# AutoGPTQ/AutoGPTQ

Measured on AMD Instinct MI355X. Metric: int4 g128 QuantLinear fwd GB/s + tokens/s, Llama-7B shapes, higher is better.
Workload: dtype f16; 1 GPU; Llama-7B linear shapes (4096->4096 x4, 4096->11008 x2, 11008->4096) x 32 blocks = 224 layers, int4 g128 no act-order, M=1 rows per step, 128 launches/step in one hipGraph (q|k|v and gate|up of a block: one gptq_forward_multi launch each); layers=224, launches=128, parallelism=single

## Files before the change

### autogptq_amd/_lib.py

```python
from __future__ import annotations

import ctypes
import os
from ctypes import POINTER, Structure, c_char_p, c_int, c_int32, c_size_t, c_void_p

import torch

_HERE = os.path.dirname(os.path.abspath(__file__))
LIB_PATH = os.environ.get("GPTQ_MI355X_LIB", os.path.join(_HERE, "libgptq_mi355x.so"))

ABI_VERSION = 8

GPTQ_F16, GPTQ_BF16, GPTQ_F32 = 0, 1, 2
ZERO_WRAP, ZERO_NOWRAP = 0, 1
EPI_NONE, EPI_SILU_MUL, EPI_GELU_TANH_MUL = 0, 1, 2
EPILOGUE_ENUM = {"none": EPI_NONE, "silu_mul": EPI_SILU_MUL, "gelu_tanh_mul": EPI_GELU_TANH_MUL}

DTYPE_ENUM = {torch.float16: GPTQ_F16, torch.bfloat16: GPTQ_BF16, torch.float32: GPTQ_F32}

EXPORTS = (
    "gptq_abi_version", "gptq_last_error", "gptq_status_string", "gptq_workspace_bytes", "gptq_workspace_bytes_ex",
    "gptq_forward", "gptq_forward_ex", "gptq_gemv", "gptq_gemm", "gptq_dequant", "gptq_grad_input",
    "gptq_unpack_weights", "gptq_unpack_zeros", "gptq_pack_weights", "gptq_pack_zeros",
    "gptq_make_sequential", "gptq_resequence_qweight", "gptq_permute_columns", "gptq_prepack_decode", "gptq_prepack_decode_bytes", "gptq_unprepack_decode",
    "gptq_awq_unpack", "gptq_awq_repack", "gptq_describe_plan",
    "gptq_init", "gptq_workspace_bytes_max", "gptq_validate_g_idx",
    "gptq_forward_multi", "gptq_workspace_bytes_multi", "gptq_forward_multi_ex", "gptq_workspace_bytes_multi_ex",
    "gptq_peer_scatter", "gptq_peer_collect", "gptq_peer_gather", "gptq_forward_scatter", "gptq_forward_gather", "gptq_peer_publish",
    "gptq_mlp_forward", "gptq_mlp_forward_ex", "gptq_mlp_forward_act", "gptq_workspace_bytes_mlp", "gptq_workspace_bytes_mlp_ex", "gptq_describe_mlp_plan",
    "gptq_moe_table_bytes", "gptq_moe_build_table", "gptq_moe_workspace_bytes", "gptq_moe_forward", "gptq_describe_moe_plan",
    "gptq_moe_decode_table_bytes", "gptq_moe_build_decode_table", "gptq_moe_decode_workspace_bytes", "gptq_moe_decode_forward", "gptq_describe_moe_decode_plan",
    "gptq_moe_batch_workspace_bytes", "gptq_moe_batch_forward", "gptq_describe_moe_batch_plan",
    "gptq_moe_prefill_workspace_bytes", "gptq_moe_prefill_forward", "gptq_describe_moe_prefill_plan",
    "gptq_moe_grad_table_bytes", "gptq_moe_build_grad_table", "gptq_moe_backward_workspace_bytes", "gptq_moe_backward", "gptq_describe_moe_backward_plan",
    "gptq_lora_down", "gptq_lora_up", "gptq_lora_apply", "gptq_describe_lora_plan",
    "gptq_lora_backward_workspace_bytes", "gptq_lora_backward", "gptq_describe_lora_backward_plan",
    "gptq_adapter_route_bytes", "gptq_adapter_route", "gptq_adapter_rows_apply", "gptq_describe_adapter_rows_plan",
    "gptq_moe_router", "gptq_describe_moe_router_plan", "gptq_moe_router_grouped", "gptq_describe_moe_router_grouped_plan",
    "gptq_moe_shared_decode_workspace_bytes", "gptq_moe_shared_decode_forward", "gptq_describe_moe_shared_decode_plan", "gptq_moe_shared_combine",
)
WS_HEADER_BYTES = 65536
STRIP_COLS = 16


class GptqLayer(Structure):
    _fields_ = [
        ("qweight", c_void_p), ("qzeros", c_void_p), ("scales", c_void_p), ("g_idx", c_void_p), ("bias", c_void_p),
        ("K", c_int32), ("N", c_int32), ("bits", c_int32), ("group_size", c_int32),
# ... 104 lines not shown
    lib.gptq_forward_multi.argtypes = [POINTER(POINTER(GptqLayer)), c_int, c_void_p, POINTER(c_void_p), c_int, c_void_p, c_size_t, c_void_p]
    lib.gptq_workspace_bytes_multi_ex.restype = c_size_t
    lib.gptq_workspace_bytes_multi_ex.argtypes = [POINTER(POINTER(GptqLayer)), c_int, c_int, POINTER(GptqTuning)]
    lib.gptq_forward_multi_ex.argtypes = lib.gptq_forward_multi.argtypes + [POINTER(GptqTuning)]
    lib.gptq_validate_g_idx.argtypes = [c_void_p, c_int, c_int]
    fw = [POINTER(GptqLayer), c_void_p, c_void_p, c_int, c_void_p, c_size_t, c_void_p]
    lib.gptq_forward.argtypes = fw
    for name in ("gptq_forward_ex", "gptq_gemv", "gptq_gemm"):
        getattr(lib, name).argtypes = fw + [POINTER(GptqTuning)]
    lib.gptq_dequant.argtypes = [POINTER(GptqLayer), c_void_p, c_void_p]
    lib.gptq_grad_input.argtypes = [POINTER(GptqLayer), c_void_p, c_void_p, c_int, c_int, c_void_p]
    lib.gptq_unpack_weights.argtypes = [c_void_p, c_int, c_int, c_int, c_void_p, c_void_p]
    lib.gptq_unpack_zeros.argtypes = [c_void_p, c_int, c_int, c_int, c_int, c_void_p, c_void_p]
    lib.gptq_pack_weights.argtypes = [c_void_p, c_void_p, c_void_p, c_void_p, c_int, c_int, c_int, c_int, c_int, c_int,
                                      c_void_p, c_void_p, c_void_p]
    lib.gptq_pack_zeros.argtypes = [c_void_p, c_int, c_int, c_int, c_int, c_void_p, c_void_p]
    lib.gptq_make_sequential.argtypes = [c_void_p, c_int, c_int, c_void_p, POINTER(c_int)]
    lib.gptq_resequence_qweight.argtypes = [c_void_p, c_void_p, c_int, c_int, c_int, c_void_p, c_void_p]
    lib.gptq_permute_columns.argtypes = [c_void_p, c_void_p, c_int, c_int, c_int, c_void_p, c_void_p]
    lib.gptq_prepack_decode_bytes.argtypes = [POINTER(GptqLayer), POINTER(c_size_t), POINTER(c_size_t)]
    lib.gptq_prepack_decode.argtypes = [POINTER(GptqLayer), c_void_p, c_void_p, c_void_p]
    lib.gptq_unprepack_decode.argtypes = [c_void_p, c_int, c_int, c_int, c_void_p, c_void_p]
    lib.gptq_describe_plan.argtypes = [POINTER(GptqLayer), c_int, POINTER(GptqTuning), c_char_p, c_size_t]
    lib.gptq_awq_unpack.argtypes = [c_void_p, c_void_p, c_void_p, c_int, c_int, c_int, c_void_p, c_void_p, c_void_p]
    lib.gptq_awq_repack.argtypes = [c_void_p, c_void_p, c_int, c_int, c_int, c_void_p, c_void_p, c_void_p]
    LP = POINTER(GptqLayer)
    lib.gptq_workspace_bytes_mlp.restype = c_size_t
    lib.gptq_workspace_bytes_mlp.argtypes = [LP, LP, LP, c_int]
    lib.gptq_workspace_bytes_mlp_ex.restype = c_size_t
    lib.gptq_workspace_bytes_mlp_ex.argtypes = [LP, LP, LP, c_int, POINTER(GptqTuning)]
    lib.gptq_mlp_forward.argtypes = [LP, LP, LP, c_void_p, c_void_p, c_int, c_void_p, c_size_t, c_void_p]
    lib.gptq_mlp_forward_ex.argtypes = lib.gptq_mlp_forward.argtypes + [POINTER(GptqTuning)]
    lib.gptq_mlp_forward_act.argtypes = [LP, LP, LP, c_int, c_void_p, c_void_p, c_int, c_void_p, c_size_t, c_void_p]
    lib.gptq_describe_mlp_plan.argtypes = [LP, LP, LP, c_int, POINTER(GptqTuning), c_char_p, c_size_t]
    MP = POINTER(GptqMoe)
    lib.gptq_moe_table_bytes.restype = c_size_t
    lib.gptq_moe_table_bytes.argtypes = [c_int]
    lib.gptq_moe_build_table.argtypes = [MP, c_void_p, c_void_p]
    lib.gptq_moe_workspace_bytes.restype = c_size_t
    lib.gptq_moe_workspace_bytes.argtypes = [MP, c_int, c_int]
    lib.gptq_moe_forward.argtypes = [MP, c_void_p, c_void_p, c_void_p, c_void_p, c_int, c_int, c_void_p, c_void_p, c_void_p, c_size_t, c_void_p]
    lib.gptq_describe_moe_plan.argtypes = [MP, c_int, c_int, c_char_p, c_size_t]
    lib.gptq_moe_decode_table_bytes.restype = c_size_t
    lib.gptq_moe_decode_table_bytes.argtypes = [c_int]
    lib.gptq_moe_build_decode_table.argtypes = [MP, c_void_p, c_void_p]
    lib.gptq_moe_decode_workspace_bytes.restype = c_size_t
# ... 106 lines not shown
def check(status: int) -> None:
    if status != 0:
        lib = load()
        msg = lib.gptq_last_error().decode("utf-8", "replace")
        kind = lib.gptq_status_string(status).decode()
        raise GptqError(status, f"gptq_mi355x: {kind}: {msg}")


def _describe(fn: str, *args) -> dict:
    buf = ctypes.create_string_buffer(512)
    check(getattr(load(), fn)(*args, buf, len(buf)))
    out = {}
    for kv in buf.value.decode().split():
        k, v = kv.split("=", 1)
        out[k] = int(v) if v.lstrip("-").isdigit() else v
    return out


def _pointer_array(ctype, items):
    return (POINTER(ctype) * max(1, len(items)))(*[ctypes.pointer(i) for i in items])


def describe_plan(layer: "GptqLayer", M: int, tuning: "GptqTuning | None" = None) -> dict:
    return _describe("gptq_describe_plan", ctypes.byref(layer), M, ctypes.byref(tuning) if tuning is not None else None)


def describe_mlp_plan(gate: "GptqLayer", up: "GptqLayer", down: "GptqLayer", M: int, tuning: "GptqTuning | None" = None) -> dict:
    return _describe("gptq_describe_mlp_plan", ctypes.byref(gate), ctypes.byref(up), ctypes.byref(down), M,
                     ctypes.byref(tuning) if tuning is not None else None)


def describe_moe_plan(moe: "GptqMoe", T: int, topk: int) -> dict:
    return _describe("gptq_describe_moe_plan", ctypes.byref(moe), T, topk)


def describe_moe_backward_plan(moe: "GptqMoe", T: int, topk: int) -> dict:
    return _describe("gptq_describe_moe_backward_plan", ctypes.byref(moe), T, topk)


def describe_moe_decode_plan(moe: "GptqMoe", T: int, topk: int) -> dict:
    return _describe("gptq_describe_moe_decode_plan", ctypes.byref(moe), T, topk)


def describe_moe_shared_decode_plan(moe: "GptqMoe", shared: "GptqMoeShared", T: int, topk: int) -> dict:
    return _describe("gptq_describe_moe_shared_decode_plan", ctypes.byref(moe), ctypes.byref(shared), T, topk)


# ... 53 lines not shown
```

### autogptq_amd/csrc/capi.hip

```cpp
#include <stdarg.h>
#include <stdio.h>
#include <string.h>

#include <algorithm>
#include <cstdlib>
#include <vector>

#include "common.cuh"
#include "launch.h"
#include "../../include/gptq_mi355x_lab.h"

using namespace gptq;

namespace {

thread_local char g_err[512] = "";

int fail(int code, const char* fmt, ...) {
    va_list ap;
    va_start(ap, fmt);
    vsnprintf(g_err, sizeof(g_err), fmt, ap);
    va_end(ap);
    return code;
}
// ... 1500 lines not shown
    if (e != hipSuccess) return hip_fail(e, "gptq_prepack_decode launch");
    return GPTQ_OK;
}

int gptq_unprepack_decode(const uint32_t* qweight_tiled, int K, int N, int bits, uint32_t* qweight_out, void* stream) {
    if (!qweight_tiled || !qweight_out) return fail(GPTQ_ERR_NULL, "qweight_tiled/qweight_out must be non-NULL");
    if (bits != 2 && bits != 3 && bits != 4 && bits != 8) return fail(GPTQ_ERR_UNSUPPORTED, "the decode copy exists for 2-, 3-, 4- and 8-bit layers (got %d)", bits);
    if (K <= 0 || N <= 0 || K % 32 || N % GPTQ_STRIP_COLS) return fail(GPTQ_ERR_SHAPE, "K (%d) must be a positive multiple of 32 and N (%d) of %d", K, N, GPTQ_STRIP_COLS);
    if ((const void*)qweight_tiled == (const void*)qweight_out) return fail(GPTQ_ERR_UNSUPPORTED, "gptq_unprepack_decode does not work in place");
    hipError_t e = launch_unprepack_decode(qweight_tiled, K, N, bits, qweight_out, (hipStream_t)stream);
    if (e != hipSuccess) return hip_fail(e, "gptq_unprepack_decode launch");
    return GPTQ_OK;
}

int gptq_permute_columns(const void* x, const int32_t* perm, int M, int K, int dtype, void* x_out, void* stream) {
    if (!x || !perm || !x_out) return fail(GPTQ_ERR_NULL, "x/perm/x_out must be non-NULL");
    if (!dtype_ok(dtype)) return fail(GPTQ_ERR_UNSUPPORTED, "unsupported dtype enum %d", dtype);
    if (M <= 0 || K <= 0) return fail(GPTQ_ERR_SHAPE, "M (%d) and K (%d) must be > 0", M, K);
    hipError_t e = launch_permute_columns(x, perm, M, K, dtype, x_out, (hipStream_t)stream);
    if (e != hipSuccess) return hip_fail(e, "gptq_permute_columns launch");
    return GPTQ_OK;
}

int gptq_describe_plan(const gptq_layer_t* L, int M, const gptq_tuning_t* tune, char* out, size_t out_bytes) {
    if (!out || out_bytes == 0) return fail(GPTQ_ERR_NULL, "out must be non-NULL");
    out[0] = 0;
    int rc = check_layer(L);
    if (rc) return rc;
    if (M <= 0) return fail(GPTQ_ERR_SHAPE, "M must be > 0, got %d", M);
    if (tune && (tune->path == 2 || tune->path == 4)) return fail(GPTQ_ERR_UNSUPPORTED, "tuning.path = %d was retired in round 6", tune->path);
    const ForwardRoute r = route_forward(L, M, tune);
    const char* separate = r.unfused_epilogue ? "separate" : "none";
    switch (r.kind) {
        case ROUTE_TILED:
        case ROUTE_TILED_PAIR: {
            const bool pair = r.kind == ROUTE_TILED_PAIR;
            snprintf(out, out_bytes, "path=gemv kernel=strips ln=4 waves=%d u=%d ksplit=%d mt=%d strips=%d pair=%d perm=0 epilogue=%s aligned=%d", r.tp.waves, r.tp.u, r.tp.ksplit, r.tp.mt,
                     r.tp.strips_total, pair ? 1 : 0, pair ? "fused" : separate, r.tp.aligned ? 1 : 0);
            break;
        }
        case ROUTE_STREAM:
        case ROUTE_STREAM_SEQ:
            snprintf(out, out_bytes, "path=gemv kernel=stream ln=%d waves=%d u=%d ksplit=%d mt=%d strips=%d pair=0 perm=%d epilogue=none", r.sp.ln, r.sp.waves,
                     r.sp.u, r.sp.ksplit, r.sp.mt, r.sp.strips_total, r.kind == ROUTE_STREAM_SEQ ? 2 : 0);
            break;
        case ROUTE_GEMM: {
// ... 126 lines not shown
```

### autogptq_amd/csrc/gemv_shared.cuh

```cuda
#pragma once
#include <type_traits>

#include "common.cuh"
#include "launch.h"

namespace gptq {

struct GemvParams {
    const unsigned* qweight;
    const unsigned* qzeros;
    const void* scales;
    const int* g_idx;
    const int* perm;
    const void* bias;
    const void* x;
    void* out;
    float* partial;
    int M, K, N, group_size, zero_mode;
    int units_total, units_per_split, chunk_units, ksplit;
    int gu_shift;
    int pair_off;
    int act;
};
hipError_t launch_gemv_generic(const gptq_layer_t& L, const GemvPlan& pl, const GemvParams& p, hipStream_t st);
// ... 62 lines not shown
template <int ROWS, bool NT>
__device__ __forceinline__ void stage_rows(__attribute__((address_space(1))) const char* const (&base)[ROWS], const unsigned (&lds)[ROWS], int tid, int w64, int step, int pieces) {
    if (w64 >= pieces) return;
    if (tid < pieces) {
#pragma unroll
        for (int r = 0; r < ROWS; ++r) dma16_sv_drop_m0<NT>(base[r], (unsigned)tid * 16u, lds[r] + (unsigned)w64 * 16u);
    }
    if (w64 + step >= pieces) return;
    if (tid + step < pieces) {
#pragma unroll
        for (int r = 0; r < ROWS; ++r) dma16_sv_drop_m0<NT>(base[r], (unsigned)(tid + step) * 16u, lds[r] + (unsigned)(w64 + step) * 16u);
    }
    if (__builtin_expect(w64 + 2 * step >= pieces, 1)) return;
    for (int a = 2 * step; w64 + a < pieces; a += step) {
        if (tid + a < pieces) {
#pragma unroll
            for (int r = 0; r < ROWS; ++r) dma16_sv_drop_m0<NT>(base[r], (unsigned)(tid + a) * 16u, lds[r] + (unsigned)(w64 + a) * 16u);
        }
    }
}
__device__ __forceinline__ int scalar_ge(int a, int b) {
    int r;
    asm("s_cmp_ge_i32 %1, %2\n\ts_cselect_b32 %0, 1, 0" : "=s"(r) : "s"(a), "s"(b) : "scc");
    return r;
}

struct GemvSeg {
    const unsigned* qweight;
    const unsigned* qzeros;
    const void* scales;
    const void* bias;
    void* out;
    int N;
    int blk_end;
    int col0;
    int pad_;
};
struct GemvStreamParams {
    GemvSeg seg[4];
    const void* x;
    unsigned long long* gran;
    unsigned* epochs;
    unsigned* err;
    int nseg, M, K, zero_mode, units_total, units_per_split, ksplit, gu_shift, nsum;
    unsigned max_spins;
};
// ... 93 lines not shown
```

### autogptq_amd/csrc/gemv_tiled.hip

```cpp
#include "gemv_tiled_kernel.cuh"
#include "../../include/gptq_mi355x_lab.h"

namespace gptq {

hipError_t launch_tiled_act(const TiledPlan& pl, const TiledParams& p, int dtype, hipStream_t st);
hipError_t init_gemv_tiled_act_device();
hipError_t launch_tiled_peer(const TiledPlan& pl, const TiledParams& p, int dtype, hipStream_t st);
hipError_t init_gemv_tiled_peer_device();
hipError_t launch_tiled_pair(const TiledPlan& pl, const TiledParams& p, int dtype, hipStream_t st);
hipError_t init_gemv_tiled_pair_device();
hipError_t launch_tiled_multi(const TiledPlan& pl, const TiledParams& p, int dtype, hipStream_t st);
hipError_t init_gemv_tiled_multi_device();

int tiled_max_waves(int u, int nstr) { return (u == 2 || nstr == 4) ? 16 : 8; }
bool tiled_has_aligned(int bits, int mt, int u, int nstr) { return bits == 4 && ((nstr == 1 && mt == 1) || (nstr == 2 && mt <= 2 && u == 4)); }
static int tiled_kpl(int bits) { return bits == 8 ? 16 : 32; }
static int tiled_chunk_bytes(int bits) { return bits == 3 ? 768 : (bits == 2 ? 512 : 1024); }
static int tiled_rec_bytes(int bits) { return bits == 8 ? 64 : 48; }

static bool tiled_pair_layer(const gptq_layer_t& L) { return is_gated(L.epilogue) && L.g_idx == nullptr && L.N % (2 * GPTQ_STRIP_COLS) == 0; }

bool tiled_layer_ok(const gptq_layer_t& L) {
    if (!L.qweight_tiled || !L.qconst_tiled || L.tiled_cols != GPTQ_STRIP_COLS || (L.epilogue != GPTQ_EPI_NONE && !tiled_pair_layer(L))) return false;
    if (L.bits != 4 && L.bits != 8 && L.bits != 3 && L.bits != 2) return false;
// ... 91 lines not shown
        else { waves = 4; u = 4; }
        if (wgs <= 128 && chunks >= 64 && pl.ksplit == 1) { waves = 8; u = 4; }
        if (pl.mt > 4) { waves = 8; u = 4; }
        if (pair && waves == 4) waves = 8;
        if (pair && waves == 8 && u == 4 && (double)((chunks + 15) / 16 * 16) / chunks - (double)((chunks + 7) / 8 * 8) / chunks >= 0.1) u = 2;
        if (nstr > 1) { waves = nstr == 4 ? 16 : 8; u = 4; }
        if (nstr == 2 && pl.mt <= 2 && A.K <= 7168) waves = 4;
        if (nstr == 2 && pl.mt == 4 && waves == 8 && (double)((chunks + 15) / 16 * 16) / chunks - (double)((chunks + 7) / 8 * 8) / chunks >= 0.1) u = 2;
        if (pl.mt == 4 && waves == 4 && !pair && nstr == 1 && ((size_t)160 * 1024 / lds_need(ks, 4)) * 4 < 12) waves = 8;
        const int per = pair ? 2 : nstr;
        while (waves > per && (waves / (2 * per)) * u >= cps) waves /= 2;
    }
    if (pair && (waves & 1)) return pl;
    if (nstr > 1 && pl.mt <= 2 && (waves > 8 || u != 4)) return pl;
    if (nstr > 1 && waves % nstr != 0) return pl;
    if (waves < 1 || waves > 16 || (u != 2 && u != 4)) return pl;
    if (waves > tiled_max_waves(u, nstr)) return pl;
    if (nstr == 4 && u == 2 && A.bits != 4) return pl;
    pl.waves = waves;
    pl.u = u;
    pl.zm2 = A.bits == 4 && A.dtype == GPTQ_BF16 && pl.mt == 2 && (long)strips * pl.ksplit < 1024;
    pl.aligned = A.K % cke == 0 && !A.g_idx && !pair && tiled_has_aligned(A.bits, pl.mt, u, nstr) &&
                 !(tune && tune->reserved[GPTQ_LAB_GEMM_VARIANT] == GPTQ_LAB_VARIANT_TILED_GENERAL);
    pl.xstride = cps * cke * 2 + 16;
    pl.lds_bytes = lds_need(pl.ksplit, waves);
    pl.xraw_off = A.g_idx ? (int)((pl.lds_bytes - ((size_t)pl.mt * ((size_t)A.K * 2 + 16) + 16) + 15) & ~(size_t)15) : 0;
    if (pl.lds_bytes > 160 * 1024) return pl;
    pl.partial_bytes = pl.ksplit > 1 ? (size_t)(pl.ksplit - 1) * M * nsum * 8 : 0;
    pl.ok = true;
    return pl;
}

hipError_t launch_tiled(const gptq_layer_t* const* Ls, const TiledPlan& pl, const void* x, void* const* outs, int M, void* ws_header, void* ws_body,
                        hipStream_t st, const gptq_peer_group_t* pg) {
    if (!pl.ok) return hipErrorInvalidValue;
    TiledParams p{};
    if (pg) {
        if (pl.nseg != 1 || pl.mt > 4 || pg->world < 1 || pg->world > GPTQ_PEER_MAX) return hipErrorInvalidValue;
        for (int r = 0; r < pg->world; ++r) {
            p.peer.xbuf[0][r] = (char*)pg->xbuf[0][r];
            p.peer.xbuf[1][r] = (char*)pg->xbuf[1][r];
            p.peer.flags[r] = pg->flags[r];
        }
        p.peer.state = pg->state;
        p.peer.world = pg->world;
        p.peer.rank = pg->rank;
// ... 15 lines not shown
    }
    const gptq_layer_t& A = *Ls[0];
    p.x = x;
    p.gran = (unsigned long long*)ws_body;
    p.epochs = ws_header ? (unsigned*)((char*)ws_header + WS_HEADER_EPOCH_OFFSET) : nullptr;
    p.err = ws_header ? (unsigned*)((char*)ws_header + WS_HEADER_BYTES - WS_HEADER_TAIL_BYTES) + 2 : nullptr;
#ifdef GPTQ_TILED_STAMPS
    if (pl.ksplit == 1) {
        const char* const e = getenv("GPTQ_TILED_STAMPS_PTR");
        p.gran = e ? (unsigned long long*)strtoull(e, nullptr, 0) : nullptr;
    }
#endif
    p.max_spins = 1u << 20;
    p.nseg = pl.nseg; p.M = M; p.K = A.K;
    p.chunks = pl.chunks_total; p.chunks_per_split = pl.chunks_per_split; p.ksplit = pl.ksplit;
    p.gu_shift = A.group_size >= A.K ? 26 : __builtin_ctz((unsigned)(A.group_size / tiled_kpl(A.bits)));
    p.nsum = pl.nsum;
    p.groups = pl.groups;
    p.xstride = pl.xstride;
    p.waves = pl.waves;
    p.xraw_off = pl.xraw_off;
    p.pair_strips = pl.pair ? A.N / (2 * GPTQ_STRIP_COLS) : 0;
    p.act = A.epilogue;
    if (pg) {
        if (A.g_idx || A.bits == 2 || (pl.u != 2 && pl.u != 4)) return hipErrorInvalidValue;
        TiledPlan plg = pl;
        plg.aligned = false;
        return launch_tiled_peer(plg, p, A.dtype, st);
    }
    if (pl.pair) return (pl.u == 2 || pl.u == 4) ? launch_tiled_pair(pl, p, A.dtype, st) : hipErrorInvalidValue;
    if (pl.nstr > 1) return (pl.u == 2 || pl.u == 4) ? launch_tiled_multi(pl, p, A.dtype, st) : hipErrorInvalidValue;
    if (A.g_idx) return launch_tiled_act(pl, p, A.dtype, st);
    return A.dtype == GPTQ_BF16 ? launch_tiled_bits<bf16, 0>(pl, p, st) : launch_tiled_bits<f16, 0>(pl, p, st);
}

hipError_t init_gemv_tiled_device() {
    hipError_t e = grant_tiled_lds<0>();
    hipError_t e2 = init_gemv_tiled_act_device();
    hipError_t e3 = init_gemv_tiled_peer_device();
    hipError_t e4 = init_gemv_tiled_pair_device();
    hipError_t e5 = init_gemv_tiled_multi_device();
    return e != hipSuccess ? e : (e2 != hipSuccess ? e2 : (e3 != hipSuccess ? e3 : (e4 != hipSuccess ? e4 : e5)));
}

}
```

### autogptq_amd/csrc/gemv_tiled_kernel.cuh

```cuda
#pragma once
#include <cstddef>

#include "gemv_shared.cuh"

namespace gptq {

struct TiledSeg {
    const void* bias;
    void* out;
    int N, col0;
};
struct PeerEpi {
    char* xbuf[2][GPTQ_PEER_MAX];
    unsigned* flags[GPTQ_PEER_MAX];
    unsigned* state;
    int world, rank;
    unsigned row_bytes, col_off_bytes, owners, pad_;
};
struct TiledParams {
    int blk_end[3];
    int act;
    const void* x;
    int M, K;
    int chunks, chunks_per_split, ksplit, gu_shift, groups, xstride, waves;
    int pair_strips;
    const unsigned* tq[4];
    const void* cst[4];
    const int* perm[4];
    int xraw_off;
    int nseg, nsum;
    unsigned max_spins;
    TiledSeg seg[4];
    unsigned long long* gran;
    unsigned* epochs;
    unsigned* err;
    PeerEpi peer;
};
static_assert(offsetof(TiledParams, perm) == 128, "the entry batch of the decode-copy kernel is the first two cache lines of its arguments");

template <int BITS> struct TiledFmt;
template <> struct TiledFmt<4> { static constexpr int WPL = 4, KPL = 32, REC = 48, ZB = 1; };
template <> struct TiledFmt<8> { static constexpr int WPL = 4, KPL = 16, REC = 64, ZB = 2; };
template <> struct TiledFmt<3> { static constexpr int WPL = 3, KPL = 32, REC = 48, ZB = 1; };
template <> struct TiledFmt<2> { static constexpr int WPL = 2, KPL = 32, REC = 48, ZB = 1; };

#ifdef GPTQ_TILED_STAMPS
#define TILED_STAMP(i) (st_[i] = __builtin_amdgcn_s_memtime() | vz_)
#define TILED_STAMPS_OUT() stamps_out()
#define TILED_HOT_END() return
#else
#define TILED_HOT_END() __builtin_amdgcn_endpgm()
#define TILED_STAMP(i) ((void)0)
#define TILED_STAMPS_OUT() ((void)0)
#endif

template <int N_> struct WordsOf { typedef unsigned type __attribute__((ext_vector_type(N_))); };

template <int BITS, int MT, int U, typename T, int MAXW, int XM = 0, int FL = 0>
__global__ void __launch_bounds__(MAXW * 64, MAXW == 16 ? 4 : 2) gemv_tiled_kernel(TiledParams p) {
    constexpr int ZM2 = FL & 1;
#ifdef GPTQ_TILED_ABL
    constexpr int ABL = GPTQ_TILED_ABL;
#else
    constexpr int ABL = 0;
#endif
    constexpr bool AL = (FL & 2) != 0 || (ABL & 1) != 0;
#ifdef GPTQ_TILED_STAMPS
    unsigned long long st_[9] = {};
    unsigned vz_;
    asm volatile("v_mov_b32 %0, 0" : "=v"(vz_));
    st_[7] = __builtin_amdgcn_s_memrealtime() | vz_;
    TILED_STAMP(0);
    auto stamps_out = [&]() {
        st_[8] = __builtin_amdgcn_s_memrealtime() | vz_;
        unsigned long long* const dbg = p.gran;
        const int b = (int)blockIdx.x, nb = (int)gridDim.x;
        const int slot = b == 0 ? 0 : (b == 1 ? 1 : (b == nb / 2 ? 2 : (b == nb - 1 ? 3 : -1)));
        if (dbg != nullptr && p.ksplit == 1 && slot >= 0 && (threadIdx.x & 63) == 0) {
#pragma unroll
            for (int i = 0; i < 9; ++i) dbg[(slot * 16 + (int)(threadIdx.x >> 6)) * 16 + i] = st_[i];
        }
    };
#endif
// ... 25 lines not shown
    const int tid = threadIdx.x, lane = tid & 63;
    const int wave = __builtin_amdgcn_readfirstlane(tid >> 6);
    const int col = lane & 15, kb = lane >> 4;
    typedef unsigned u32x16 __attribute__((ext_vector_type(16)));
    typedef unsigned long long u64x8 __attribute__((ext_vector_type(8)));
    typedef unsigned long long u64x4 __attribute__((ext_vector_type(4)));
    static_assert(offsetof(TiledParams, x) == 16 && offsetof(TiledParams, M) == 24 && offsetof(TiledParams, chunks) == 32 && offsetof(TiledParams, pair_strips) == 60 &&
                  offsetof(TiledParams, tq) == 64 && offsetof(TiledParams, cst) == 96 && offsetof(TiledParams, perm) == 128 && offsetof(TiledParams, xraw_off) == 160 && offsetof(TiledParams, act) == 12, "the entry batch");
    u32x16 ha;
    u64x8 hb;
    [[maybe_unused]] u64x4 hp = {};
    [[maybe_unused]] int xraw_off = 0;
    {
        const auto kargs = __builtin_amdgcn_kernarg_segment_ptr();
        if constexpr (ACT)
            asm volatile("s_load_dwordx16 %0, %4, 0x0\n\ts_load_dwordx16 %1, %4, 0x40\n\ts_load_dwordx8 %2, %4, 0x80\n\ts_load_dword %3, %4, 0xa0\n\ts_waitcnt lgkmcnt(0)"
                         : "=&s"(ha), "=&s"(hb), "=&s"(hp), "=&s"(xraw_off) : "s"(kargs));
        else
            asm volatile("s_load_dwordx16 %0, %2, 0x0\n\ts_load_dwordx16 %1, %2, 0x40\n\ts_waitcnt lgkmcnt(0)" : "=&s"(ha), "=&s"(hb) : "s"(kargs));
    }
    const int be0 = (int)ha[0], be1 = (int)ha[1], be2 = (int)ha[2], Mrows = (int)ha[6], K = (int)ha[7], nchunks = (int)ha[8], cps = (int)ha[9], ksplit = (int)ha[10],
              gshift = (int)ha[11], G = (int)ha[12], xstride = (int)ha[13], W = (int)ha[14];
    [[maybe_unused]] const int hstrips = (int)ha[15], act = (int)ha[3];
    typedef __attribute__((address_space(1))) const char gchar;
    gchar* const xg = (gchar*)(((unsigned long long)ha[5] << 32) | ha[4]);
    int sidx = blockIdx.x, ks = 0, cb = 0, ce = nchunks, kbeg = 0, kend = K;
    if (__builtin_expect(ksplit != 1, 0)) {
        sidx = (int)blockIdx.x / ksplit; ks = (int)blockIdx.x - sidx * ksplit;
        cb = ks * cps; ce = min(cb + cps, nchunks);
        kbeg = cb * CKE; kend = min(ce * CKE, K);
    }
    unsigned long long tqs_ = hb[0], csts_ = hb[4];
    [[maybe_unused]] unsigned long long perm_ = hp[0];
    int sbase = 0, s = 0;
    if constexpr (ACT)
        asm("s_cmp_ge_i32 %[i], %[e0]\n\ts_cbranch_scc0 1f\n\t"
            "s_mov_b64 %[tq], %[tq1]\n\ts_mov_b64 %[cs], %[cs1]\n\ts_mov_b64 %[pm], %[pm1]\n\ts_mov_b32 %[sb], %[e0]\n\ts_mov_b32 %[s], 1\n\t"
            "s_cmp_ge_i32 %[i], %[e1]\n\ts_cselect_b64 %[tq], %[tq2], %[tq]\n\ts_cselect_b64 %[cs], %[cs2], %[cs]\n\ts_cselect_b64 %[pm], %[pm2], %[pm]\n\ts_cselect_b32 %[sb], %[e1], %[sb]\n\ts_cselect_b32 %[s], 2, %[s]\n\t"
            "s_cmp_ge_i32 %[i], %[e2]\n\ts_cselect_b64 %[tq], %[tq3], %[tq]\n\ts_cselect_b64 %[cs], %[cs3], %[cs]\n\ts_cselect_b64 %[pm], %[pm3], %[pm]\n\ts_cselect_b32 %[sb], %[e2], %[sb]\n\ts_cselect_b32 %[s], 3, %[s]\n"
            "1:"
            : [tq] "+&s"(tqs_), [cs] "+&s"(csts_), [pm] "+&s"(perm_), [sb] "+&s"(sbase), [s] "+&s"(s)
            : [i] "s"(sidx), [e0] "s"(be0), [e1] "s"(be1), [e2] "s"(be2), [tq1] "s"(hb[1]), [tq2] "s"(hb[2]), [tq3] "s"(hb[3]), [cs1] "s"(hb[5]), [cs2] "s"(hb[6]), [cs3] "s"(hb[7]),
              [pm1] "s"(hp[1]), [pm2] "s"(hp[2]), [pm3] "s"(hp[3])
            : "scc");
    else
        asm("s_cmp_ge_i32 %[i], %[e0]\n\ts_cbranch_scc0 1f\n\t"
// ... 12 lines not shown
    const int sel = NSTR == 1 ? 0 : (scalar_ge(wave, Wh) + (NSTR == 4 ? scalar_ge(wave, 2 * Wh) + scalar_ge(wave, 3 * Wh) : 0));
    const int wv = NSTR == 1 ? wave : wave - sel * Wh;
    const int strip_w = PAIR ? strip + sel * hstrips : (MULTI ? strip * NSTR + sel : strip);
    char* const xs = smem;
    char* const cs = smem + (size_t)MT * xstride;
    const unsigned crec = (unsigned)G * (unsigned)REC;
    const size_t cpad = ((size_t)crec + 15) & ~(size_t)15;
    float* const red = (float*)(cs + NSTR * cpad);
    gchar* const tb = tqs + (size_t)(unsigned)strip_w * ((unsigned)nchunks * (unsigned)CHB);
    gchar* const cg = csts + (size_t)(unsigned)(MULTI ? strip * NSTR : strip) * crec;
    const unsigned t_lane = (unsigned)lane * (WPL * 4u);
    [[maybe_unused]] unsigned tlv = t_lane;
    auto stage_all = [&]() __attribute__((always_inline)) {
        const unsigned xs_lds = (unsigned)(size_t)(__attribute__((address_space(3))) char*)xs, cs_lds = (unsigned)(size_t)(__attribute__((address_space(3))) char*)cs;
        const int w64 = wave * 64, step = W * 64;
        gchar* xrow[MT];
        unsigned xdst[MT];
        if constexpr (XM == 0 || XM == 3 || XM == 4 || MULTI) {
#pragma unroll
            for (int m = 0; m < MT; ++m) {
                xrow[m] = xg + (unsigned)((m == 0 ? 0 : min(m, Mrows - 1)) * K + kbeg) * 2u;
                xdst[m] = xs_lds + m * xstride;
            }
            stage_rows<MT, false>(xrow, xdst, tid, w64, step, (kend - kbeg) >> 3);
        } else if constexpr (ACT) {
#pragma unroll
            for (int m = 0; m < MT; ++m) {
                xrow[m] = xg + (unsigned)((m == 0 ? 0 : min(m, Mrows - 1)) * K) * 2u;
                xdst[m] = xs_lds + (unsigned)xraw_off + m * (K * 2 + 16);
            }
            stage_rows<MT, false>(xrow, xdst, tid, w64, step, K >> 3);
        }
        const int cpieces = (int)(crec >> 4) * (MULTI ? NSTR : 1);
        if constexpr (PAIR) {
            gchar* const crow[2] = {cg, cg + (size_t)(unsigned)hstrips * crec};
            const unsigned cdst[2] = {cs_lds, cs_lds + (unsigned)cpad};
            stage_rows<2, true>(crow, cdst, tid, w64, step, cpieces);
        } else {
            gchar* const crow[1] = {cg};
            const unsigned cdst[1] = {cs_lds};
            stage_rows<1, true>(crow, cdst, tid, w64, step, cpieces);
        }
    };
#ifndef GPTQ_TILED_WEIGHTS_FIRST
    stage_all();
#endif
    typedef int i32x4 __attribute__((ext_vector_type(4)));
    i32x4 pa[2][2] = {};
    const int apieces = ACT ? (kend - kbeg) >> 3 : 0;
    if constexpr (ACT) {
        const int* const pg = permp + kbeg;
        if (tid < apieces) { pa[0][0] = *(const i32x4*)(pg + tid * 8); pa[0][1] = *(const i32x4*)(pg + tid * 8 + 4); }
        if (tid + W * 64 < apieces) { pa[1][0] = *(const i32x4*)(pg + (tid + W * 64) * 8); pa[1][1] = *(const i32x4*)(pg + (tid + W * 64) * 8 + 4); }
    }
    auto x_gather = [&]() {
        const int* const pg = permp + kbeg;
        const char* const xraw = smem + xraw_off;
        for (int pc0 = tid; pc0 < apieces; pc0 += 2 * W * 64) {
            const int pcb = pc0 + W * 64;
            const bool two = pcb < apieces;
            if (pc0 != tid) {
                pa[0][0] = *(const i32x4*)(pg + pc0 * 8); pa[0][1] = *(const i32x4*)(pg + pc0 * 8 + 4);
                if (two) { pa[1][0] = *(const i32x4*)(pg + pcb * 8); pa[1][1] = *(const i32x4*)(pg + pcb * 8 + 4); }
            }
// ... 122 lines not shown
        if constexpr (AL) {
            const unsigned long long sb0 = (unsigned long long)tb + (unsigned long long)((unsigned)min(c, ce - 1) * (unsigned)CHB);
            const unsigned long long sb = ((unsigned long long)(unsigned)__builtin_amdgcn_readfirstlane((int)(sb0 >> 32)) << 32) | (unsigned)__builtin_amdgcn_readfirstlane((int)(unsigned)sb0);
            asm volatile("" : "+v"(tlv));
            return __builtin_nontemporal_load((const __attribute__((address_space(1))) qvec*)((gchar*)sb + tlv));
        } else {
            return __builtin_nontemporal_load((const __attribute__((address_space(1))) qvec*)(tb + ((unsigned)min(c, ce - 1) * (unsigned)CHB + t_lane)));
        }
    };
    auto first_pass = [&]() __attribute__((always_inline)) {
        TILED_STAMP(1);
        seg_request();
#ifdef GPTQ_TILED_WEIGHTS_FIRST
        stage_all();
        asm volatile("s_waitcnt vmcnt(0)" ::: "memory");
#else
        asm volatile("s_waitcnt vmcnt(%0)" ::"n"(U) : "memory");
#endif
        if constexpr (ACT) {
            __syncthreads();
            x_gather();
        }
        __syncthreads();
        if constexpr (XC) x_to_f16();
        if constexpr (XS) x_sums();
        seg_pin();
        if (biasp != nullptr && tid < NE && n_t < (PAIR ? N >> 1 : N)) {
            bv0 = DType<T>::to_f32(((const gT*)biasp)[n_t]);
            if constexpr (PAIR) bv1 = DType<T>::to_f32(((const gT*)biasp)[n_t + (N >> 1)]);
        }
        TILED_STAMP(2);
        staged = true;
    };
    auto chunk = [&](auto steady_c, const int cj, [[maybe_unused]] const int j, const qvec qv) __attribute__((always_inline)) {
        constexpr bool STEADY = AL && decltype(steady_c)::value;
        const int cc = STEADY ? cj : min(cj, ce - 1);
        bool live;
        unsigned short sraw;
        unsigned z;
        u32x4 xa[NX];
        u32x4 xb[MT > 4 ? NX : 1];
        if constexpr (AL) {
            live = cj < ce;
            const unsigned go = (unsigned)((cc * 4) >> gshift) * (unsigned)REC;
            sraw = *(const __attribute__((address_space(3))) unsigned short*)(sl + go);
            if constexpr (F::ZB == 1) z = *(const __attribute__((address_space(3))) unsigned char*)(zl + go);
// ... 132 lines not shown
        }
    };
#ifdef GPTQ_TILED_NO_ROLL
    for (int cbase = cb; cbase < ce; cbase += Wh * U) {
        const int c0 = cbase + wv * U;
        qvec q[U];
#pragma unroll
        for (int j = 0; j < U; ++j) q[j] = wload(c0 + j);
        if (!staged) first_pass();
#ifdef GPTQ_TILED_STAMPS
        if (cbase + Wh * U >= ce) { asm volatile("s_waitcnt vmcnt(0)" ::: "memory"); TILED_STAMP(3); }
#endif
#pragma unroll
        for (int j = 0; j < U; ++j) chunk(std::false_type{}, c0 + j, j, q[j]);
    }
#else
    if (cb < ce) {
        int c0 = cb + wv * U;
        qvec q[U];
#pragma unroll
        for (int j = 0; j < U; ++j) q[j] = wload(c0 + j);
        first_pass();
        if constexpr (AL) { xpass = (unsigned)(size_t)xll + (unsigned)(c0 - cb) * (unsigned)(CKE * 2); asm volatile("" : "+v"(xpass)); }
        for (int cn = c0 + Wh * U; cn < ce; cn += Wh * U) {
#pragma unroll
            for (int j = 0; j < U; ++j) {
                chunk(std::true_type{}, c0 + j, j, q[j]);
                __builtin_amdgcn_sched_barrier(0);
                q[j] = wload(cn + j);
                __builtin_amdgcn_sched_barrier(0);
            }
            c0 = cn;
            if constexpr (AL) { xpass += (unsigned)(Wh * U) * (unsigned)(CKE * 2); asm volatile("" : "+v"(xpass)); }
        }
#ifdef GPTQ_TILED_STAMPS
        asm volatile("s_waitcnt vmcnt(0)" ::: "memory"); TILED_STAMP(3);
#endif
#pragma unroll
        for (int j = 0; j < U; ++j) chunk(std::false_type{}, c0 + j, j, q[j]);
    }
#endif
    TILED_STAMP(4);
#pragma unroll
    for (int m = 0; m < MT; ++m) acc[m] = kslot_sum_swap(acc[m]);
    if (__builtin_expect(!staged, 0)) {
        seg_request();
        seg_pin();
        __syncthreads();
    }
    gT* const outg = (gT*)outp;
    if (lane < 16) {
#pragma unroll
        for (int m = 0; m < MT; ++m) red[wave * ES + m * 16 + lane] = acc[m];
    }
    __syncthreads();
    TILED_STAMP(5);
// ... 182 lines not shown
```

### autogptq_amd/csrc/launch.h

```cpp
#pragma once
#include <hip/hip_runtime.h>
#include <stddef.h>
#include "../../include/gptq_mi355x.h"

namespace gptq {

struct GemvPlan {
    int ln, waves, ksplit, strips, mt, mtiles;
    int units_total, units_per_split, chunk_units;
    bool perk, use_seq;
    bool mfma;
    bool mfmag;
    bool magic;
    bool pair;
    bool xperm;
    size_t xperm_bytes;
    int u;
    size_t lds_bytes, workspace_bytes;
};
GemvPlan plan_gemv(const gptq_layer_t& L, int M, const gptq_tuning_t* tune);
hipError_t launch_gemv(const gptq_layer_t& L, const GemvPlan& pl, const void* x, void* out, int M,
                       void* workspace, hipStream_t st);

struct MidPlan {
// ... 89 lines not shown
constexpr size_t WS_HEADER_EPOCH_OFFSET = 32768;
constexpr size_t WS_HEADER_TAIL_BYTES = 64;
struct StreamPlan {
    bool ok;
    int nseg, ln, waves, u, mt, ksplit, units_total, units_per_split, strips_total, nsum;
    size_t lds_bytes;
    size_t partial_bytes;
};
StreamPlan plan_stream(const gptq_layer_t* const* layers, int n, int M, const gptq_tuning_t* tune);
hipError_t launch_stream(const gptq_layer_t* const* layers, const StreamPlan& pl, const void* x, void* const* outs, int M,
                         void* ws_header, void* ws_body, hipStream_t st);
Stream64Plan plan_stream64(const gptq_layer_t* const* layers, int n, int M, const gptq_tuning_t* tune);
hipError_t launch_stream64(const gptq_layer_t* const* layers, const Stream64Plan& pl, const void* x, void* const* outs, int M,
                           void* ws_header, void* partial, const uint32_t* qweight_override, hipStream_t st);
struct TiledPlan {
    bool ok;
    int nstr;
    bool pair;
    int nseg, bits, waves, u, mt, ksplit, chunks_total, chunks_per_split, strips_total, nsum, groups, xstride, xraw_off;
    size_t lds_bytes;
    size_t partial_bytes;
    bool zm2;
    bool aligned;
};
bool tiled_layer_ok(const gptq_layer_t& L);
TiledPlan plan_tiled(const gptq_layer_t* const* layers, int n, int M, const gptq_tuning_t* tune);
hipError_t launch_tiled(const gptq_layer_t* const* layers, const TiledPlan& pl, const void* x, void* const* outs, int M, void* ws_header, void* ws_body,
                        hipStream_t st, const gptq_peer_group_t* pg = nullptr);
hipError_t init_gemv_tiled_device();
size_t tiled_weight_bytes(const gptq_layer_t& L);
size_t tiled_const_bytes(const gptq_layer_t& L);
hipError_t launch_prepack_decode(const uint32_t* qweight, const uint32_t* qzeros, const void* scales, int K, int N, int bits, int group_size, int zero_mode,
                                 uint32_t* tiled_out, void* const_out, hipStream_t st);
hipError_t launch_unprepack_decode(const uint32_t* tiled, int K, int N, int bits, uint32_t* qweight_out, hipStream_t st);
bool stream_preferred(const gptq_layer_t& L, int M);
bool multi_preferred(const gptq_layer_t* const* layers, int n, int M);
hipError_t launch_silu_mul2(const void* g, const void* u, void* out, size_t total, int dtype, int act, hipStream_t st);
bool silu_mul2_permute_ok(int K, int dtype);
hipError_t launch_silu_mul2_permute(const void* g, const void* u, const int32_t* perm, int M, int K, int dtype, int act, void* out, hipStream_t st);
hipError_t init_mlp_device();
bool wide_gemm_ok(const gptq_layer_t& L, int M, bool use_seq, bool xslot_glds);
hipError_t launch_gemm_wide(const gptq_layer_t& L, const uint32_t* qweight, const void* x, void* out, int M, bool glds, hipStream_t st, bool tiled = false);
bool wide_sk_ok(const gptq_layer_t& L, int M);
bool wide_sk_pays(const gptq_layer_t& L, int M);
WideSkGeom wide_sk_geom(const gptq_layer_t& L, int M);
hipError_t launch_gemm_wide_sk(const gptq_layer_t& L, const void* x, void* out, int M, void* ws_header, void* slots, hipStream_t st);
// ... 166 lines not shown
```

### include/gptq_mi355x.h

```cpp
#ifndef GPTQ_MI355X_H
#define GPTQ_MI355X_H

#include <stddef.h>
#include <stdint.h>

#ifdef __cplusplus
extern "C" {
#endif

#define GPTQ_MI355X_ABI_VERSION 8
#define GPTQ_WORKSPACE_HEADER_BYTES 65536

typedef enum gptq_status_t {
    GPTQ_OK = 0,
    GPTQ_ERR_NULL = 1,
    GPTQ_ERR_SHAPE = 2,
    GPTQ_ERR_UNSUPPORTED = 3,
    GPTQ_ERR_WORKSPACE = 4,
    GPTQ_ERR_LAUNCH = 5
} gptq_status_t;

typedef enum gptq_dtype_t { GPTQ_F16 = 0, GPTQ_BF16 = 1, GPTQ_F32 = 2 } gptq_dtype_t;

typedef enum gptq_zero_mode_t { GPTQ_ZERO_WRAP = 0, GPTQ_ZERO_NOWRAP = 1 } gptq_zero_mode_t;
// ... 185 lines not shown
                            int dtype, int flags, float *logits_out, float *scores_out, int64_t *topk_idx, float *topk_w, void *stream);
int gptq_describe_moe_router_grouped_plan(int T, int H, int E, int topk, int n_group, int topk_group, int dtype, int flags, char *out, size_t out_bytes);

int gptq_unpack_weights(const uint32_t *qweight, int K, int N, int bits, uint8_t *w_out, void *stream);
int gptq_unpack_zeros(const uint32_t *qzeros, int G, int N, int bits, int zero_mode, int32_t *z_out, void *stream);

int gptq_pack_weights(const void *W, const void *scale_in, const void *zero_in, const int32_t *g_idx,
                      int K, int N, int bits, int group_size, int w_dtype, int qparam_dtype,
                      uint32_t *qweight_out, void *scales_out, void *stream);
int gptq_pack_zeros(const void *zero_in, int G, int N, int bits, int qparam_dtype,
                    uint32_t *qzeros_out, void *stream);

int gptq_make_sequential(const int32_t *g_idx_host, int K, int group_size,
                         int32_t *perm_out_host, int *uniform_out);
int gptq_validate_g_idx(const int32_t *g_idx_host, int K, int G);
int gptq_resequence_qweight(const uint32_t *qweight, const int32_t *perm, int K, int N, int bits,
                            uint32_t *qweight_seq_out, void *stream);
int gptq_prepack_decode_bytes(const gptq_layer_t *layer, size_t *tiled_bytes, size_t *const_bytes);
int gptq_prepack_decode(const gptq_layer_t *layer, uint32_t *qweight_tiled_out, void *qconst_tiled_out, void *stream);
int gptq_unprepack_decode(const uint32_t *qweight_tiled, int K, int N, int bits, uint32_t *qweight_out, void *stream);
int gptq_permute_columns(const void *x, const int32_t *perm, int M, int K, int dtype, void *x_out, void *stream);

int gptq_describe_plan(const gptq_layer_t *layer, int M, const gptq_tuning_t *tuning, char *out, size_t out_bytes);

int gptq_awq_unpack(const uint32_t *awq_qweight, const uint32_t *awq_qzeros, const void *awq_scales, int K, int N,
                    int group_size, void *weight_kn_out, int8_t *zeros_out, void *stream);
int gptq_awq_repack(const uint32_t *awq_qweight, const uint32_t *awq_qzeros, int K, int N, int group_size,
                    uint32_t *qweight_out, uint32_t *qzeros_out, void *stream);

#define GPTQ_PEER_MAX 8
typedef struct gptq_peer_group_t {
    void     *xbuf[2][GPTQ_PEER_MAX];
    uint32_t *flags[GPTQ_PEER_MAX];
    uint32_t *state;
    int32_t world, rank;
    int32_t rows_max, N;
} gptq_peer_group_t;

int gptq_peer_scatter(const gptq_peer_group_t *pg, const void *y_local, int M, int n_local, int dtype, void *stream);
int gptq_peer_collect(const gptq_peer_group_t *pg, void *out, int M, int dtype, uint32_t max_spins, void *stream);
int gptq_peer_gather(const gptq_peer_group_t *pg, const void *y_local, void *out, int M, int n_local, int dtype,
                     uint32_t max_spins, void *stream);
int gptq_forward_scatter(const gptq_layer_t *layer, const void *x, int M, const gptq_peer_group_t *pg, void *workspace, size_t workspace_bytes,
                         void *stream);
int gptq_forward_gather(const gptq_layer_t *layer, const void *x, void *out, int M, const gptq_peer_group_t *pg, uint32_t max_spins, void *workspace,
                        size_t workspace_bytes, void *stream);
// ... 7 lines not shown
```

### include/gptq_mi355x_lab.h

```cpp
#ifndef GPTQ_MI355X_LAB_H
#define GPTQ_MI355X_LAB_H

#define GPTQ_LAB_DEPTH 0

#define GPTQ_LAB_OPT 1
#define GPTQ_LAB_OPT_FIELD_DECODE 1
#define GPTQ_LAB_OPT_MID_XREG 1
#define GPTQ_LAB_OPT_MID_GRANULES 3
#define GPTQ_LAB_OPT_GEMM_BK32 32

#define GPTQ_LAB_GEMM_KERNEL 2
#define GPTQ_LAB_GEMM_SKINNY 1
#define GPTQ_LAB_GEMM_TILED 2
#define GPTQ_LAB_GEMM_STRIP16 3
#define GPTQ_LAB_GEMM_STREAM64 4
#define GPTQ_LAB_GEMM_MID 5

#define GPTQ_LAB_GEMM_VARIANT 3
#define GPTQ_LAB_VARIANT_PLAIN_LOOP 1
#define GPTQ_LAB_VARIANT_SETPRIO 2
#define GPTQ_LAB_VARIANT_CROSS_STEP 3
#define GPTQ_LAB_VARIANT_REG_STAGED_X 5
#define GPTQ_LAB_VARIANT_ONE_K_GROUP 6
#define GPTQ_LAB_VARIANT_TWO_K_GROUPS 7
#define GPTQ_LAB_VARIANT_TAIL_ON 40
#define GPTQ_LAB_VARIANT_TAIL_OFF 41
#define GPTQ_LAB_VARIANT_TAIL_NO_LIMIT 42
#define GPTQ_LAB_VARIANT_WIDE_OFF 44
#define GPTQ_LAB_VARIANT_WIDE_ON 45
#define GPTQ_LAB_VARIANT_WIDE_ROWS 46
#define GPTQ_LAB_VARIANT_WIDE_ROWS_ON 47
#define GPTQ_LAB_VARIANT_WIDE_SK_ON 48
#define GPTQ_LAB_VARIANT_WIDE_SK_OFF 49
#define GPTQ_LAB_VARIANT_ROWS_ON 50
#define GPTQ_LAB_VARIANT_ROWS_OFF 51
#define GPTQ_LAB_VARIANT_PANEL_ON 52
#define GPTQ_LAB_VARIANT_PANEL_OFF 53
#define GPTQ_LAB_VARIANT_MLP_TWO_PASSES 54
#define GPTQ_LAB_VARIANT_TILED_GENERAL 60

#endif
```

Before: 3935 GB/s.

## Stage tiled-kernel activations and constants in two steps to start weight loop earlier

In the tiled GEMV kernel for f16 int4 single-strip layers without g_idx, only the first slice of x and the matching group constants is staged into LDS before the first barrier. The rest is staged afterwards, while the first pass of weight chunks runs, and a mid-loop waitcnt plus barrier syncs before the later chunks use it. The aim is to shorten the prologue latency before weight streaming begins in the M=1 decode kernels. It adds a second barrier, reuses the pair_strips field through a union, and adds a describe hook plus a variant to turn the feature off.

```diff
diff --git a/autogptq_amd/_lib.py b/autogptq_amd/_lib.py
--- a/autogptq_amd/_lib.py
+++ b/autogptq_amd/_lib.py
@@ -23,7 +23,7 @@
     "gptq_forward", "gptq_forward_ex", "gptq_gemv", "gptq_gemm", "gptq_dequant", "gptq_grad_input",
     "gptq_unpack_weights", "gptq_unpack_zeros", "gptq_pack_weights", "gptq_pack_zeros",
     "gptq_make_sequential", "gptq_resequence_qweight", "gptq_permute_columns", "gptq_prepack_decode", "gptq_prepack_decode_bytes", "gptq_unprepack_decode",
-    "gptq_awq_unpack", "gptq_awq_repack", "gptq_describe_plan",
+    "gptq_awq_unpack", "gptq_awq_repack", "gptq_describe_plan", "gptq_describe_plan_xstage",
     "gptq_init", "gptq_workspace_bytes_max", "gptq_validate_g_idx",
     "gptq_forward_multi", "gptq_workspace_bytes_multi", "gptq_forward_multi_ex", "gptq_workspace_bytes_multi_ex",
     "gptq_peer_scatter", "gptq_peer_collect", "gptq_peer_gather", "gptq_forward_scatter", "gptq_forward_gather", "gptq_peer_publish",
@@ -174,6 +174,7 @@
     lib.gptq_prepack_decode.argtypes = [POINTER(GptqLayer), c_void_p, c_void_p, c_void_p]
     lib.gptq_unprepack_decode.argtypes = [c_void_p, c_int, c_int, c_int, c_void_p, c_void_p]
     lib.gptq_describe_plan.argtypes = [POINTER(GptqLayer), c_int, POINTER(GptqTuning), c_char_p, c_size_t]
+    lib.gptq_describe_plan_xstage.argtypes = [POINTER(GptqLayer), c_int, POINTER(GptqTuning)]
     lib.gptq_awq_unpack.argtypes = [c_void_p, c_void_p, c_void_p, c_int, c_int, c_int, c_void_p, c_void_p, c_void_p]
     lib.gptq_awq_repack.argtypes = [c_void_p, c_void_p, c_int, c_int, c_int, c_void_p, c_void_p, c_void_p]
     LP = POINTER(GptqLayer)
@@ -326,7 +327,11 @@
 
 
 def describe_plan(layer: "GptqLayer", M: int, tuning: "GptqTuning | None" = None) -> dict:
-    return _describe("gptq_describe_plan", ctypes.byref(layer), M, ctypes.byref(tuning) if tuning is not None else None)
+    tp = ctypes.byref(tuning) if tuning is not None else None
+    d = _describe("gptq_describe_plan", ctypes.byref(layer), M, tp)
+    if d.get("kernel") == "strips":
+        d["xstage"] = int(load().gptq_describe_plan_xstage(ctypes.byref(layer), M, tp))
+    return d
 
 
 def describe_mlp_plan(gate: "GptqLayer", up: "GptqLayer", down: "GptqLayer", M: int, tuning: "GptqTuning | None" = None) -> dict:
diff --git a/autogptq_amd/csrc/capi.hip b/autogptq_amd/csrc/capi.hip
--- a/autogptq_amd/csrc/capi.hip
+++ b/autogptq_amd/csrc/capi.hip
@@ -1546,6 +1546,12 @@
     return GPTQ_OK;
 }
 
+int gptq_describe_plan_xstage(const gptq_layer_t* L, int M, const gptq_tuning_t* tune) {
+    if (check_layer(L) || M <= 0 || (tune && (tune->path == 2 || tune->path == 4))) return 0;
+    const ForwardRoute r = route_forward(L, M, tune);
+    return (r.kind == ROUTE_TILED || r.kind == ROUTE_TILED_PAIR) ? r.tp.xsteps : 0;
+}
+
 int gptq_describe_plan(const gptq_layer_t* L, int M, const gptq_tuning_t* tune, char* out, size_t out_bytes) {
     if (!out || out_bytes == 0) return fail(GPTQ_ERR_NULL, "out must be non-NULL");
     out[0] = 0;
diff --git a/autogptq_amd/csrc/gemv_shared.cuh b/autogptq_amd/csrc/gemv_shared.cuh
--- a/autogptq_amd/csrc/gemv_shared.cuh
+++ b/autogptq_amd/csrc/gemv_shared.cuh
@@ -108,6 +108,12 @@
 __device__ __forceinline__ int scalar_ge(int a, int b) {
     int r;
     asm("s_cmp_ge_i32 %1, %2\n\ts_cselect_b32 %0, 1, 0" : "=s"(r) : "s"(a), "s"(b) : "scc");
+    return r;
+}
+
+__device__ __forceinline__ int scalar_sel_nz(unsigned c, int a, int b) {
+    int r;
+    asm("s_cmp_lg_u32 %1, 0\n\ts_cselect_b32 %0, %2, %3" : "=s"(r) : "s"(c), "s"(a), "s"(b) : "scc");
     return r;
 }
 
diff --git a/autogptq_amd/csrc/gemv_tiled.hip b/autogptq_amd/csrc/gemv_tiled.hip
--- a/autogptq_amd/csrc/gemv_tiled.hip
+++ b/autogptq_amd/csrc/gemv_tiled.hip
@@ -137,6 +137,8 @@
     pl.zm2 = A.bits == 4 && A.dtype == GPTQ_BF16 && pl.mt == 2 && (long)strips * pl.ksplit < 1024;
     pl.aligned = A.K % cke == 0 && !A.g_idx && !pair && tiled_has_aligned(A.bits, pl.mt, u, nstr) &&
                  !(tune && tune->reserved[GPTQ_LAB_GEMM_VARIANT] == GPTQ_LAB_VARIANT_TILED_GENERAL);
+    pl.xsteps = (!A.g_idx && !pair && nstr == 1 && A.bits == 4 && A.dtype == GPTQ_F16 && pl.ksplit == 1 && A.K > waves * u * cke &&
+                 !(tune && tune->reserved[GPTQ_LAB_GEMM_VARIANT] == GPTQ_LAB_VARIANT_TILED_ONE_STEP)) ? 2 : 1;
     pl.xstride = cps * cke * 2 + 16;
     pl.lds_bytes = lds_need(pl.ksplit, waves);
     pl.xraw_off = A.g_idx ? (int)((pl.lds_bytes - ((size_t)pl.mt * ((size_t)A.K * 2 + 16) + 16) + 15) & ~(size_t)15) : 0;
@@ -198,6 +200,12 @@
     p.xraw_off = pl.xraw_off;
     p.pair_strips = pl.pair ? A.N / (2 * GPTQ_STRIP_COLS) : 0;
     p.act = A.epilogue;
+    if (pl.xsteps == 2 && !pg && !pl.pair) {
+        const int kpl = tiled_kpl(A.bits), k1 = pl.waves * pl.u * 4 * kpl;
+        const int gt = (((k1 - 1) / kpl) >> p.gu_shift) + 1, g1 = gt < pl.groups ? gt : pl.groups;
+        const unsigned xp = (unsigned)k1 / 8u, cp = (unsigned)g1 * (unsigned)tiled_rec_bytes(A.bits) / 16u;
+        if (k1 < A.K && xp < 65536u && cp < 65536u) p.xstep1 = xp | (cp << 16);
+    }
     if (pg) {
         if (A.g_idx || A.bits == 2 || (pl.u != 2 && pl.u != 4)) return hipErrorInvalidValue;
         TiledPlan plg = pl;
diff --git a/autogptq_amd/csrc/gemv_tiled_kernel.cuh b/autogptq_amd/csrc/gemv_tiled_kernel.cuh
--- a/autogptq_amd/csrc/gemv_tiled_kernel.cuh
+++ b/autogptq_amd/csrc/gemv_tiled_kernel.cuh
@@ -23,7 +23,10 @@
     const void* x;
     int M, K;
     int chunks, chunks_per_split, ksplit, gu_shift, groups, xstride, waves;
-    int pair_strips;
+    union {
+        int pair_strips;
+        unsigned xstep1;
+    };
     const unsigned* tq[4];
     const void* cst[4];
     const int* perm[4];
@@ -59,6 +62,7 @@
 template <int BITS, int MT, int U, typename T, int MAXW, int XM = 0, int FL = 0>
 __global__ void __launch_bounds__(MAXW * 64, MAXW == 16 ? 4 : 2) gemv_tiled_kernel(TiledParams p) {
     constexpr int ZM2 = FL & 1;
+    constexpr bool BF_ = std::is_same_v<T, bf16>;
 #ifdef GPTQ_TILED_ABL
     constexpr int ABL = GPTQ_TILED_ABL;
 #else
@@ -130,6 +134,12 @@
     const int be0 = (int)ha[0], be1 = (int)ha[1], be2 = (int)ha[2], Mrows = (int)ha[6], K = (int)ha[7], nchunks = (int)ha[8], cps = (int)ha[9], ksplit = (int)ha[10],
               gshift = (int)ha[11], G = (int)ha[12], xstride = (int)ha[13], W = (int)ha[14];
     [[maybe_unused]] const int hstrips = (int)ha[15], act = (int)ha[3];
+#if defined(GPTQ_TILED_NO_ROLL) || defined(GPTQ_TILED_WEIGHTS_FIRST)
+    constexpr bool TWO = false;
+#else
+    constexpr bool TWO = XM == 0 && BITS == 4 && !BF_;
+#endif
+    [[maybe_unused]] const unsigned xstep1 = TWO ? ha[15] : 0u;
     typedef __attribute__((address_space(1))) const char gchar;
     gchar* const xg = (gchar*)(((unsigned long long)ha[5] << 32) | ha[4]);
     int sidx = blockIdx.x, ks = 0, cb = 0, ce = nchunks, kbeg = 0, kend = K;
@@ -188,7 +198,13 @@
                 xrow[m] = xg + (unsigned)((m == 0 ? 0 : min(m, Mrows - 1)) * K + kbeg) * 2u;
                 xdst[m] = xs_lds + m * xstride;
             }
-            stage_rows<MT, false>(xrow, xdst, tid, w64, step, (kend - kbeg) >> 3);
+#ifdef GPTQ_TILED_STAGE1
+            stage_rows<MT, false>(xrow, xdst, tid, w64, step, min(kend - kbeg, Wh * U * CKE) >> 3);
+#else
+            int xpieces = (kend - kbeg) >> 3;
+            if constexpr (TWO) xpieces = scalar_sel_nz(xstep1, (int)(xstep1 & 0xffffu), xpieces);
+            stage_rows<MT, false>(xrow, xdst, tid, w64, step, xpieces);
+#endif
         } else if constexpr (ACT) {
 #pragma unroll
             for (int m = 0; m < MT; ++m) {
@@ -197,7 +213,12 @@
             }
             stage_rows<MT, false>(xrow, xdst, tid, w64, step, K >> 3);
         }
-        const int cpieces = (int)(crec >> 4) * (MULTI ? NSTR : 1);
+#ifdef GPTQ_TILED_STAGE1
+        const int cpieces = (ACT ? G : min(G, ((min(kend - kbeg, Wh * U * CKE) - 1) >> LKPL >> gshift) + 1)) * (REC >> 4) * (MULTI ? NSTR : 1);
+#else
+        int cpieces = (int)(crec >> 4) * (MULTI ? NSTR : 1);
+        if constexpr (TWO) cpieces = scalar_sel_nz(xstep1, (int)(xstep1 >> 16), cpieces);
+#endif
         if constexpr (PAIR) {
             gchar* const crow[2] = {cg, cg + (size_t)(unsigned)hstrips * crec};
             const unsigned cdst[2] = {cs_lds, cs_lds + (unsigned)cpad};
@@ -206,6 +227,25 @@
             gchar* const crow[1] = {cg};
             const unsigned cdst[1] = {cs_lds};
             stage_rows<1, true>(crow, cdst, tid, w64, step, cpieces);
+        }
+    };
+    auto stage_rest = [&]() __attribute__((always_inline)) {
+        if constexpr (TWO) {
+            const unsigned xs_lds = (unsigned)(size_t)(__attribute__((address_space(3))) char*)xs, cs_lds = (unsigned)(size_t)(__attribute__((address_space(3))) char*)cs;
+            const int w64 = wave * 64, step = W * 64;
+            const int xp1 = (int)(xstep1 & 0xffffu), cp1 = (int)(xstep1 >> 16);
+            const int xp2 = (K >> 3) - xp1, cp2 = (int)(crec >> 4) - cp1;
+            gchar* xrow[MT];
+            unsigned xdst[MT];
+#pragma unroll
+            for (int m = 0; m < MT; ++m) {
+                xrow[m] = xg + ((unsigned)((m == 0 ? 0 : min(m, Mrows - 1)) * K) * 2u + (unsigned)xp1 * 16u);
+                xdst[m] = xs_lds + m * xstride + (unsigned)xp1 * 16u;
+            }
+            stage_rows<MT, false>(xrow, xdst, tid, w64, step, xp2);
+            gchar* const crow[1] = {cg + (unsigned)cp1 * 16u};
+            const unsigned cdst[1] = {cs_lds + (unsigned)cp1 * 16u};
+            stage_rows<1, true>(crow, cdst, tid, w64, step, cp2);
         }
     };
 #ifndef GPTQ_TILED_WEIGHTS_FIRST
@@ -374,6 +414,9 @@
             x_gather();
         }
         __syncthreads();
+        if constexpr (TWO) {
+            if (__builtin_expect(xstep1 != 0u, 0)) stage_rest();
+        }
         if constexpr (XC) x_to_f16();
         if constexpr (XS) x_sums();
         seg_pin();
@@ -552,16 +595,36 @@
         for (int j = 0; j < U; ++j) q[j] = wload(c0 + j);
         first_pass();
         if constexpr (AL) { xpass = (unsigned)(size_t)xll + (unsigned)(c0 - cb) * (unsigned)(CKE * 2); asm volatile("" : "+v"(xpass)); }
-        for (int cn = c0 + Wh * U; cn < ce; cn += Wh * U) {
-#pragma unroll
-            for (int j = 0; j < U; ++j) {
-                chunk(std::true_type{}, c0 + j, j, q[j]);
-                __builtin_amdgcn_sched_barrier(0);
-                q[j] = wload(cn + j);
-                __builtin_amdgcn_sched_barrier(0);
-            }
-            c0 = cn;
-            if constexpr (AL) { xpass += (unsigned)(Wh * U) * (unsigned)(CKE * 2); asm volatile("" : "+v"(xpass)); }
+        int cn = c0 + Wh * U;
+        auto steady = [&](const int stop) __attribute__((always_inline)) {
+            for (; cn < stop; cn += Wh * U) {
+#pragma unroll
+                for (int j = 0; j < U; ++j) {
+                    chunk(std::true_type{}, c0 + j, j, q[j]);
+                    __builtin_amdgcn_sched_barrier(0);
+                    q[j] = wload(cn + j);
+                    __builtin_amdgcn_sched_barrier(0);
+                }
+                c0 = cn;
+                if constexpr (AL) { xpass += (unsigned)(Wh * U) * (unsigned)(CKE * 2); asm volatile("" : "+v"(xpass)); }
+            }
+        };
+        if constexpr (TWO) {
+            int stop = ce, pend = 0;
+            if (__builtin_expect(xstep1 != 0u, 0)) {
+                pend = 1; stop = min(cn + 1, ce);
+                if (cn >= ce) asm volatile("s_waitcnt vmcnt(0)" ::: "memory");
+            }
+        second_run:
+            asm volatile("" : "+s"(stop), "+s"(pend));
+            steady(stop);
+            if (__builtin_expect(pend != 0, 0)) {
+                asm volatile("s_waitcnt vmcnt(%0)\n\ts_barrier" ::"n"(U) : "memory");
+                pend = 0; stop = ce;
+                goto second_run;
+            }
+        } else {
+            steady(ce);
         }
 #ifdef GPTQ_TILED_STAMPS
         asm volatile("s_waitcnt vmcnt(0)" ::: "memory"); TILED_STAMP(3);
diff --git a/autogptq_amd/csrc/launch.h b/autogptq_amd/csrc/launch.h
--- a/autogptq_amd/csrc/launch.h
+++ b/autogptq_amd/csrc/launch.h
@@ -135,6 +135,7 @@
     size_t partial_bytes;
     bool zm2;
     bool aligned;
+    int xsteps;
 };
 bool tiled_layer_ok(const gptq_layer_t& L);
 TiledPlan plan_tiled(const gptq_layer_t* const* layers, int n, int M, const gptq_tuning_t* tune);
diff --git a/include/gptq_mi355x.h b/include/gptq_mi355x.h
--- a/include/gptq_mi355x.h
+++ b/include/gptq_mi355x.h
@@ -231,6 +231,7 @@
 int gptq_permute_columns(const void *x, const int32_t *perm, int M, int K, int dtype, void *x_out, void *stream);
 
 int gptq_describe_plan(const gptq_layer_t *layer, int M, const gptq_tuning_t *tuning, char *out, size_t out_bytes);
+int gptq_describe_plan_xstage(const gptq_layer_t *layer, int M, const gptq_tuning_t *tuning);
 
 int gptq_awq_unpack(const uint32_t *awq_qweight, const uint32_t *awq_qzeros, const void *awq_scales, int K, int N,
                     int group_size, void *weight_kn_out, int8_t *zeros_out, void *stream);
diff --git a/include/gptq_mi355x_lab.h b/include/gptq_mi355x_lab.h
--- a/include/gptq_mi355x_lab.h
+++ b/include/gptq_mi355x_lab.h
@@ -38,5 +38,6 @@
 #define GPTQ_LAB_VARIANT_PANEL_OFF 53
 #define GPTQ_LAB_VARIANT_MLP_TWO_PASSES 54
 #define GPTQ_LAB_VARIANT_TILED_GENERAL 60
+#define GPTQ_LAB_VARIANT_TILED_ONE_STEP 61
 
 #endif
```

Result: faster. 3974 GB/s (median of 6 runs) (+1.0%).
